# BlaineHeffron/WaveformML

Measured on AMD Instinct MI355X. Metric: waveforms/sec (LitPSD sparse-conv training step), higher is better.
Workload: dtype bf16; 1 GPU; SubMConv3d PSD net, 14x11 PMT grid x 256 samples, Cin=2 Cout=32, 256 events/rank/step, rulebook rebuilt every step; active_voxels_per_rank=84164, global_batch=256, parallelism=dp1, execution=hipgraph

## Files before the change

include/wfsparse.h:

```cpp
#ifndef WFSPARSE_H
#define WFSPARSE_H

#include <stddef.h>
#include <stdint.h>

#ifdef __cplusplus
extern "C" {
#endif

#define WFS_OK 0
#define WFS_EINVAL 1
#define WFS_EOVERFLOW 2
#define WFS_EHIP 3
#define WFS_EWORKSPACE 4

#define WFS_F32 0
#define WFS_BF16 1
#define WFS_F16 2

#define WFS_MAX_DIM 4

#define WFS_ABI_VERSION 6
int wfs_abi_version(void);
const char *wfs_last_error(void);
// ... 146 lines not shown

int wfs_to_dense_bwd_mapped(const void *dY, const uint32_t *ticket, const int32_t *slot_id, int64_t M,
                            const int64_t *m_dev, int32_t batch_size, int64_t V, int32_t C, void *dX, int32_t dtype,
                            void *stream);

int wfs_sparse_head_ok(int32_t batch, int64_t V, int32_t C, int32_t O, int32_t dtype);
size_t wfs_sparse_head_workspace_bytes(int32_t batch, int64_t V, int32_t C, int32_t O);
int wfs_sparse_head_fwd(const void *X, const uint32_t *ticket, const int32_t *slot_id, int64_t M,
                        const int64_t *m_dev, int32_t batch, int64_t V, int32_t C, const float *W,
                        const float *bias, int32_t O, float *Y, int32_t dtype, void *workspace,
                        size_t workspace_bytes, void *stream);
int wfs_sparse_head_bwd(const void *X, const float *G, const uint32_t *ticket, const int32_t *slot_id,
                        int64_t M, const int64_t *m_dev, int32_t batch, int64_t V, int32_t C, const float *W,
                        int32_t O, void *dX, float *dW, float *dB, int32_t dtype, void *workspace,
                        size_t workspace_bytes, wfs_dw_job *defer, void *stream);

size_t wfs_head_workspace_bytes(int64_t B, int64_t I, int32_t O);

int wfs_head_fwd(const void *X, int64_t B, int64_t I, const float *W, const float *bias, int32_t O,
                 float *Y, int32_t dtype, void *stream);

int wfs_head_bwd(const void *X, const float *G, int64_t B, int64_t I, const float *W, int32_t O,
                 void *dX, float *dW, float *dB, int32_t dtype, void *workspace, size_t workspace_bytes,
                 wfs_dw_job *defer, void *stream);



size_t wfs_tcn_lds_bytes(int32_t L, int32_t levels, int32_t backward);

int wfs_tcn_fwd(const void *X, int64_t N, int32_t L, const float *taps, const float *bias, int32_t levels,
// ... 86 lines not shown
```

waveformml_amd/_lib.py:

```python
import ctypes
import os

import torch

_HERE = os.path.dirname(os.path.abspath(__file__))
LIB_PATH = os.environ.get("WFS_LIB") or os.path.join(_HERE, "lib", "libwfsparse.so")

WFS_OK, WFS_EINVAL, WFS_EOVERFLOW, WFS_EHIP, WFS_EWORKSPACE = 0, 1, 2, 3, 4
WFS_F32, WFS_BF16, WFS_F16 = 0, 1, 2
WFS_MAX_DIM = 4
WFS_RNN_RELU, WFS_RNN_TANH = 0, 1
WFS_ABI_VERSION = 6
TIMER_GATHER_CONV, TIMER_GATHER_DW, TIMER_RULEBOOK, TIMER_CONV_BACKWARD = 0, 1, 2, 3

c_i32p = ctypes.POINTER(ctypes.c_int32)
c_i64p = ctypes.POINTER(ctypes.c_int64)
_vp, _i32, _i64, _sz = ctypes.c_void_p, ctypes.c_int32, ctypes.c_int64, ctypes.c_size_t


class Geometry(ctypes.Structure):
    _fields_ = [("ndim", _i32), ("batch_size", _i32), ("subm", _i32), ("K", _i32),
                ("spatial", _i32 * WFS_MAX_DIM), ("out_shape", _i32 * WFS_MAX_DIM),
                ("ksize", _i32 * WFS_MAX_DIM), ("stride", _i32 * WFS_MAX_DIM),
                ("padding", _i32 * WFS_MAX_DIM), ("dilation", _i32 * WFS_MAX_DIM),
# ... 57 lines not shown
                                       _i32, _vp, _vp, _vp, _vp, _sz, _i32, _vp, _vp]),
    "wfs_bn_relu_bwd": (ctypes.c_int, [_vp, _vp, _i64, _i32, _vp, _vp, _vp, _vp, _i32, _i32, _vp, _vp, _vp, _vp, _sz,
                                       _i32, _vp, _vp]),
    "wfs_rulebook_cell_map": (ctypes.c_int, [ctypes.POINTER(Geometry), _i64, _vp, ctypes.POINTER(_vp), ctypes.POINTER(_vp),
                                             c_i64p]),
    "wfs_to_dense_mapped": (ctypes.c_int, [_vp, _vp, _vp, _i64, _vp, _i32, _i64, _i32, _vp, _i32, _vp]),
    "wfs_to_dense_bwd_mapped": (ctypes.c_int, [_vp, _vp, _vp, _i64, _vp, _i32, _i64, _i32, _vp, _i32, _vp]),
    "wfs_to_dense": (ctypes.c_int, [_vp, _vp, _i64, _i32, c_i32p, _i32, _i32, _vp, _vp, _i32, _vp, _vp]),
    "wfs_to_dense_bwd": (ctypes.c_int, [_vp, _vp, _i64, _i32, c_i32p, _i32, _i32, _vp, _i32, _vp, _vp]),
    "wfs_sparse_head_ok": (ctypes.c_int, [_i32, _i64, _i32, _i32, _i32]),
    "wfs_sparse_head_workspace_bytes": (_sz, [_i32, _i64, _i32, _i32]),
    "wfs_sparse_head_fwd": (ctypes.c_int, [_vp, _vp, _vp, _i64, _vp, _i32, _i64, _i32, _vp, _vp, _i32, _vp, _i32, _vp, _sz,
                                           _vp]),
    "wfs_sparse_head_bwd": (ctypes.c_int, [_vp, _vp, _vp, _vp, _i64, _vp, _i32, _i64, _i32, _vp, _i32, _vp, _vp, _vp, _i32,
                                           _vp, _sz, ctypes.POINTER(DwJob), _vp]),
    "wfs_head_workspace_bytes": (_sz, [_i64, _i64, _i32]),
    "wfs_head_fwd": (ctypes.c_int, [_vp, _i64, _i64, _vp, _vp, _i32, _vp, _i32, _vp]),
    "wfs_head_bwd": (ctypes.c_int, [_vp, _vp, _i64, _i64, _vp, _i32, _vp, _vp, _vp, _i32, _vp, _sz, ctypes.POINTER(DwJob),
                                    _vp]),
    "wfs_tcn_lds_bytes": (_sz, [_i32, _i32, _i32]),
    "wfs_tcn_taps_fwd": (ctypes.c_int, [_vp, _i32, _i32, _vp, _vp, _vp]),
    "wfs_tcn_taps_bwd": (ctypes.c_int, [_vp, _i32, _i32, _vp, _i64, _vp]),
    "wfs_tcn_fwd": (ctypes.c_int, [_vp, _i64, _i32, _vp, _vp, _i32, _i32, _vp, _i32, ctypes.c_float, _vp, _vp]),
    "wfs_tcn_bwd": (ctypes.c_int, [_vp, _vp, _i64, _i32, _vp, _vp, _i32, _i32, _vp, _vp, _i32, ctypes.c_float, _vp,
                                    _vp]),
    "wfs_tcnc_ok": (ctypes.c_int, [_i32, c_i32p, _i32, _i32, _i32, _i32]),
    "wfs_tcnc_n_conv": (ctypes.c_int, [_i32, c_i32p, _i32, _i32]),
    "wfs_tcnc_weights_floats": (_sz, [_i32, c_i32p, _i32, _i32]),
    "wfs_tcnc_saved_floats": (_sz, [_i64, _i32, _i32, c_i32p, _i32]),
    "wfs_tcnc_bwd_workspace_floats": (_sz, [_i64, _i32, _i32, c_i32p, _i32, _i32]),
# ... 113 lines not shown
```

waveformml_amd/csrc/head.hip:

```cpp
#include "wfs_common.h"

namespace {
constexpr int TB = 256;
constexpr int MAXO = 8;

template <typename T>
__device__ __forceinline__ void load8(const T *p, float *v) {
    if constexpr (sizeof(T) == 4) {
        float4 a = *reinterpret_cast<const float4 *>(p), b = *reinterpret_cast<const float4 *>(p + 4);
        v[0] = a.x; v[1] = a.y; v[2] = a.z; v[3] = a.w; v[4] = b.x; v[5] = b.y; v[6] = b.z; v[7] = b.w;
    } else {
        uint4 u = *reinterpret_cast<const uint4 *>(p);
        wfs_unpack2<T>(u.x, v[0], v[1]);
        wfs_unpack2<T>(u.y, v[2], v[3]);
        wfs_unpack2<T>(u.z, v[4], v[5]);
        wfs_unpack2<T>(u.w, v[6], v[7]);
    }
}
template <typename T>
__device__ __forceinline__ void store8(T *p, const float *v) {
    if constexpr (sizeof(T) == 4) {
        *reinterpret_cast<float4 *>(p) = make_float4(v[0], v[1], v[2], v[3]);
        *reinterpret_cast<float4 *>(p + 4) = make_float4(v[4], v[5], v[6], v[7]);
    } else {
// ... 165 lines not shown
            for (int w = 0; w < TB / 64; ++w) v += sdb[w][threadIdx.x];
            dB[threadIdx.x] = v;
        }
    }
    long long e = (long long)blockIdx.x * TB + threadIdx.x;
    if (e >= OI) return;
    float s = 0.f;
    for (int c = 0; c < nchunk; ++c) s += part[(long long)c * OI + e];
    dW[e] = s;
}

int head_chunks(long long B) {
    long long c = (B + 31) / 32;
    return (int)(c < 1 ? 1 : (c > 16 ? 16 : c));
}
constexpr int XE_TB = 1024;
__global__ void __launch_bounds__(XE_TB) k_xent_mean(const float *__restrict__ Z, const long long *__restrict__ target,
                                                     long long B, int C, long long ignore_index,
                                                     float *__restrict__ loss, float *__restrict__ dZ) {
    __shared__ float sL[XE_TB];
    __shared__ float sN[XE_TB];
    float l = 0.f, n = 0.f;
    for (long long b = threadIdx.x; b < B; b += XE_TB) {
        const long long t = target[b];
        if (t == ignore_index || t < 0 || t >= C) continue;
        const float *z = Z + b * C;
        float m = z[0];
        for (int c = 1; c < C; ++c) m = fmaxf(m, z[c]);
        float se = 0.f;
        for (int c = 0; c < C; ++c) se += expf(z[c] - m);
        l += (m + logf(se)) - z[t];
        n += 1.f;
    }
    sL[threadIdx.x] = l;
    sN[threadIdx.x] = n;
    __syncthreads();
    for (int w = XE_TB / 2; w > 0; w >>= 1) {
        if ((int)threadIdx.x < w) {
            sL[threadIdx.x] += sL[threadIdx.x + w];
            sN[threadIdx.x] += sN[threadIdx.x + w];
        }
        __syncthreads();
    }
    const float cnt = sN[0];
    if (threadIdx.x == 0) *loss = sL[0] / cnt;
    if (!dZ) return;
    const float inv = cnt > 0.f ? 1.f / cnt : 0.f;
    for (long long b = threadIdx.x; b < B; b += XE_TB) {
        const long long t = target[b];
        const float *z = Z + b * C;
        float *d = dZ + b * C;
        if (t == ignore_index || t < 0 || t >= C) {
            for (int c = 0; c < C; ++c) d[c] = 0.f;
            continue;
        }
        float m = z[0];
        for (int c = 1; c < C; ++c) m = fmaxf(m, z[c]);
        float se = 0.f;
        for (int c = 0; c < C; ++c) se += expf(z[c] - m);
        const float r = inv / se;
        for (int c = 0; c < C; ++c) d[c] = expf(z[c] - m) * r - (c == t ? inv : 0.f);
    }
}

template <typename T, int O>
__global__ void __launch_bounds__(64) k_head_fwd_any(const T *__restrict__ X, const float *__restrict__ W,
                                                     const float *__restrict__ bias, float *__restrict__ Y, long long I) {
    const long long b = blockIdx.x;
    const int lane = threadIdx.x;
    float acc[O];
#pragma unroll
    for (int o = 0; o < O; ++o) acc[o] = 0.f;
    for (long long i = lane; i < I; i += 64) {
        const float x = wfs_ld(X + b * I + i);
#pragma unroll
        for (int o = 0; o < O; ++o) acc[o] = fmaf(x, W[o * I + i], acc[o]);
    }
// ... 188 lines not shown
```

waveformml_amd/csrc/shead.hip:

```cpp
#include <stdlib.h>

#include "wfs_common.h"

namespace {

constexpr int SH_CELLS = 64;
constexpr int SH_EVENTS = 16;

__device__ __forceinline__ long long valid_rows(long long R, const long long *r_dev) {
    long long v = r_dev ? *r_dev : R;
    return v < R ? v : R;
}

__device__ __forceinline__ void store8(float *p, const float *x) {
    *(float4 *)p = float4{x[0], x[1], x[2], x[3]};
    *(float4 *)(p + 4) = float4{x[4], x[5], x[6], x[7]};
}
template <typename H>
__device__ __forceinline__ void store8(H *p, const float *x) {
    uint4 v;
    v.x = wfs_pack2<H>(x[0], x[1]);
    v.y = wfs_pack2<H>(x[2], x[3]);
    v.z = wfs_pack2<H>(x[4], x[5]);
    v.w = wfs_pack2<H>(x[6], x[7]);
// ... 85 lines not shown
            for (int l = 0; l < 64; ++l) s += sT[l * TS + lane];
            sP[(cg * SH_EVENTS + e0) * O + lane] = s;
        }
        __builtin_amdgcn_wave_barrier();
    }
    __syncthreads();
    if (threadIdx.x < SH_EVENTS * O) {
        const int e = threadIdx.x / O;
        const int b = slice * SH_EVENTS + e;
        float s = 0.f;
        for (int g = 0; g < ncg; ++g) s += sP[g * SH_EVENTS * O + threadIdx.x];
        if (b < B) part[((long long)tile * B + b) * O + (threadIdx.x % O)] = s;
    }
}

__global__ void __launch_bounds__(256) k_shead_sum(const float *__restrict__ part, int ntiles, int B, int O,
                                                   const float *__restrict__ bias, float *__restrict__ Y) {
    const int i = blockIdx.x * 256 + threadIdx.x;
    if (i >= B * O) return;
    float s = bias ? bias[i % O] : 0.f;
    for (int t0 = 0; t0 < ntiles; t0 += 8) {
        float v[8];
#pragma unroll
        for (int t = 0; t < 8; ++t) v[t] = part[(long long)(t0 + t < ntiles ? t0 + t : ntiles - 1) * B * O + i];
#pragma unroll
        for (int t = 0; t < 8; ++t) s += t0 + t < ntiles ? v[t] : 0.f;
    }
    Y[i] = s;
}

template <typename H, int O>
__global__ void __launch_bounds__(512) k_shead_bwd(const H *__restrict__ X, const float *__restrict__ G,
                                                    const unsigned *__restrict__ ticket, const int *__restrict__ slot,
                                                    long long M, const long long *__restrict__ m_dev, int B, int V, int C,
                                                    const float *__restrict__ W, H *__restrict__ dX,
                                                    float *__restrict__ part, float *__restrict__ dB) {
    const int lane = threadIdx.x & 63, cg = threadIdx.x >> 6;
    const int tile = blockIdx.x, slice = blockIdx.y;
    const int cell = tile * SH_CELLS + lane;
    const bool in = cell < V;
    const int cc = in ? cell : V - 1;
    const long long Mv = valid_rows(M, m_dev);
    float w[O][8];
    if (dX) {
#pragma unroll
        for (int o = 0; o < O; ++o)
#pragma unroll
            for (int j = 0; j < 8; ++j) w[o][j] = W[((long long)o * C + cg * 8 + j) * V + cc];
    }
    int row[SH_EVENTS];
#pragma unroll
    for (int e = 0; e < SH_EVENTS; ++e) {
        const int b = slice * SH_EVENTS + e;
        const long long at = (long long)(b < B ? b : B - 1) * V + cc;
        const unsigned t = ticket[at];
        const int r = slot[at];
        row[e] = (in && b < B && t != 0xFFFFFFFFu && r >= 0 && r < Mv) ? r : -1;
    }
    float acc[O][8];
#pragma unroll
    for (int o = 0; o < O; ++o)
#pragma unroll
        for (int j = 0; j < 8; ++j) acc[o][j] = 0.f;
    constexpr int SH_BATCH = ShBatch<H>::n;
#pragma unroll
    for (int e0 = 0; e0 < SH_EVENTS; e0 += SH_BATCH) {
        Piece<H> q[SH_BATCH];
        float g[SH_BATCH][O];
#pragma unroll
        for (int i = 0; i < SH_BATCH; ++i) {
            if (part) q[i] = load_piece<H>(X + (long long)(row[e0 + i] >= 0 ? row[e0 + i] : 0) * C + cg * 8);
            const int b = slice * SH_EVENTS + e0 + i;
#pragma unroll
            for (int o = 0; o < O; ++o) g[i][o] = G[(long long)(b < B ? b : B - 1) * O + o];
        }
#pragma unroll
        for (int i = 0; i < SH_BATCH; ++i) {
            const int e = e0 + i;
            const bool act = row[e] >= 0;
            if (part) {
                float x[8];
                widen<H>(q[i], x);
#pragma unroll
                for (int o = 0; o < O; ++o) {
                    const float go = act ? g[i][o] : 0.f;
#pragma unroll
                    for (int j = 0; j < 8; ++j) acc[o][j] = fmaf(go, x[j], acc[o][j]);
                }
            }
            if (dX && act) {
                float d[8];
#pragma unroll
                for (int j = 0; j < 8; ++j) {
                    float t = 0.f;
#pragma unroll
                    for (int o = 0; o < O; ++o) t = fmaf(g[i][o], w[o][j], t);
                    d[j] = t;
                }
                store8(dX + (long long)row[e] * C + cg * 8, d);
            }
        }
    }
    if (part && in) {
        float *dst = part + (long long)slice * O * C * V;
#pragma unroll
        for (int o = 0; o < O; ++o)
#pragma unroll
            for (int j = 0; j < 8; ++j) dst[((long long)o * C + cg * 8 + j) * V + cell] = acc[o][j];
    }
    if (dB && tile == 0 && slice == 0 && cg == 0) {
#pragma unroll
        for (int o = 0; o < O; ++o) {
            float s = 0.f;
            for (int b = lane; b < B; b += 64) s += G[(long long)b * O + o];
#pragma unroll
            for (int d = 32; d >= 1; d >>= 1) s += __shfl_xor(s, d, 64);
            if (lane == 0) dB[o] = s;
        }
    }
}

inline size_t fwd_lds(int waves, int O) { return ((size_t)waves * 64 * ((8 * O) | 1) + (size_t)waves * SH_EVENTS * O) * sizeof(float); }
inline int sh_tiles(long long V) { return (int)wfs_cdiv(V, SH_CELLS); }
inline int sh_slices(int B) { return (int)wfs_cdiv(B, SH_EVENTS); }

}

extern "C" int wfs_sparse_head_ok(int32_t batch, int64_t V, int32_t C, int32_t O, int32_t dtype) {
    return batch >= 1 && batch <= 65535 * SH_EVENTS && V >= 1 && V < (1ll << 24) && C >= 8 && C <= 64 && C % 8 == 0 &&
           O >= 1 && O <= 4 && wfs_dtype_ok(dtype) && (long long)O * C * V < (1ll << 31) && (long long)batch * V < (1ll << 31);
}

extern "C" size_t wfs_sparse_head_workspace_bytes(int32_t batch, int64_t V, int32_t C, int32_t O) {
    const size_t fwd = (size_t)sh_tiles(V) * (size_t)batch * O * sizeof(float);
// ... 54 lines not shown
#define WFS_SHB(T)                                                                                                      \
    WFS_SH_DISPATCH(O, (k_shead_bwd<T, OO><<<grid, block, 0, stream>>>((const T *)X, G, ticket, slot_id, M, md, batch, (int)V, \
                                                                        C, W, (T *)dX, part, dB)))
    if (dtype == WFS_F32) { WFS_SHB(float); } else if (dtype == WFS_BF16) { WFS_SHB(wfs_bf16); } else { WFS_SHB(wfs_f16); }
#undef WFS_SHB
    WFS_LAUNCH_CHECK();
    if (!dW) return WFS_OK;
    const long long per = (long long)O * C * V;
    const wfs_dw_job job = {part, sh_slices(batch), per, 1, 1, 1, 0, dW};
    if (defer) {
        *defer = job;
        return WFS_OK;
    }
    return wfs_launch_dw_jobs(&job, 1, stream);
}
```

waveformml_amd/psd/lit.py:

```python
import logging

import torch
from torch import nn

from .config import DictionaryUtility, ModuleUtility


class LitPSD(nn.Module):
    def __init__(self, config, trial=None):
        super().__init__()
        self.trial = trial
        self.pylog = logging.getLogger(__name__)
        self.config = config
        self.n_type = config.system_config.n_type
        self.lr = config.optimize_config.lr
        self.modules_util = ModuleUtility(config.net_config.imports + config.dataset_config.imports +
                                          config.optimize_config.imports)
        self.model = self.modules_util.retrieve_class(config.net_config.net_class)(config)
        criterion_class = self.modules_util.retrieve_class(config.net_config.criterion_class)
        self.criterion = criterion_class(*config.net_config.criterion_params, reduction="mean")
        self.occlude_index = getattr(config.dataset_config, "occlude_index", None)
        self.softmax = nn.LogSoftmax(dim=1)
        self.logged = {}
        self.optimizer_parameters = None
# ... 40 lines not shown
            if not hasattr(oc, "scheduler_params"):
                raise IOError("Optimizer config has a learning scheduler class specified. You must also set "
                              "lr_schedule_parameters (dictionary of key value pairs).")
            scheduler = self.modules_util.retrieve_class(oc.scheduler_class)(
                optimizer, **DictionaryUtility.to_dict(oc.scheduler_params))
            return [optimizer], [scheduler]
        return optimizer

    def _loss(self, predictions, target):
        if predictions.is_cuda:
            from ..spconv import functional as Fsp
            if Fsp.can_fuse_cross_entropy(self.criterion, predictions, target):
                return Fsp.cross_entropy_mean(predictions, target, self.criterion.ignore_index)
        return self.criterion.forward(predictions, target)

    def training_step(self, batch, batch_idx):
        c, f, n_valid, target = self._unpack(batch)
        predictions = self._predict(c, f, target, n_valid)
        loss = self._loss(predictions, target)
        self.log("train_loss", loss, on_epoch=True, prog_bar=True, logger=True)
        return loss

    def validation_step(self, batch, batch_idx):
        c, f, n_valid, target = self._unpack(batch)
        predictions = self._predict(c, f, target, n_valid)
        loss = self.criterion.forward(predictions, target)
        pred = torch.argmax(self.softmax(predictions), dim=1)
        acc = (pred == target).float().mean()
        results = {"val_loss": loss, "val_acc": acc}
        self.log_dict(results, on_epoch=True, prog_bar=True, logger=True)
        return results

    def test_step(self, batch, batch_idx):
        c, f, n_valid, target = self._unpack(batch)
# ... 10 lines not shown
```

waveformml_amd/psd/net.py:

```python
import logging

import torch
from torch import nn

from .blocks import LinearBlock, SparseConv2DBlock, SparseConv2DPreserve
from .config import DictionaryUtility, ModuleUtility


class SPConvPreserveNet(nn.Module):

    def __init__(self, config):
        super().__init__()
        self.log = logging.getLogger(__name__)
        self.system_config = config.system_config
        self.net_config = config.net_config
        self.nsamples = self.system_config.n_samples
        self.ntype = self.system_config.n_type
        self.modules_util = ModuleUtility(self.net_config.imports)
        if "spconv" in self.modules_util.modules:
            self.spconv = self.modules_util.modules["spconv"]
        else:
            import waveformml_amd.spconv as sp
            self.spconv = sp
        hparams = DictionaryUtility.to_dict(self.net_config.hparams.conv_params)
# ... 34 lines not shown
        self.batch_size_hint = None
        self.batch_events = None
        self._build()
        net_type = getattr(self.net_config, "net_type", "2DConvolution")
        if net_type == "3DConvolution":
            self.ndim = 3
            self.spatial_size = [14, 11, int(self.nsamples)]
            self.register_buffer("permute_tensor", torch.LongTensor([3, 0, 1, 2]), persistent=False)
        else:
            if net_type != "2DConvolution":
                self.log.warning("Warning: unknown net_type in net_config: {}".format(net_type))
            self.ndim = 2
            self.spatial_size = [14, 11]
            self.register_buffer("permute_tensor", torch.LongTensor([2, 0, 1]), persistent=False)

    def forward(self, x, batch_size=None):
        coords, feats = x[0], x[1]
        if hasattr(self, "waveformLayer"):
            feats = self.waveformLayer(feats.unsqueeze(1)).squeeze(1)
        if batch_size is None:
            batch_size = getattr(self, "batch_size_hint", None)
        if batch_size is None:
            batch_size = int(coords[-1, -1]) + 1
        handed = getattr(self, "batch_first_indices", None)
        if handed is not None and handed[0] is coords:
            indices = handed[1]
        else:
            make = lambda: coords[:, self.permute_tensor].contiguous()
            reused = getattr(getattr(self.spconv, "ops", None), "reused", None)
            indices = reused("batch_first", coords, make) if reused is not None else make()
        st = self.spconv.SparseConvTensor(feats, indices, self.spatial_size,
                                          batch_size)
        if len(x) > 2 and x[2] is not None:
            st.n_valid = x[2]
        ev = getattr(self, "batch_events", None)
        if ev is not None and ev[0] is coords and handed is not None and handed[0] is coords:
            st.events = ev[1]
        return self._head(st)

    def _head(self, st):
        fsp = getattr(self.spconv, "functional", None)
        if fsp is not None and hasattr(fsp, "sparse_head") and hasattr(self.sparseModel, "run"):
            layers = list(self.linear)
            out = self.sparseModel.run(st, list(self.sparseModel._modules.values()), stop_before_dense=True)
            if hasattr(out, "features") and hasattr(out, "dense"):
                if fsp.can_use_sparse_head(out, layers):
                    self.head_route = "sparse_head"
                    return fsp.sparse_head(out, layers[0])
                out = out.dense()
        else:
            out = self.sparseModel(st)
        self.head_route = "dense"
        out = out.view(-1, self.n_linear)
        if fsp is not None and hasattr(fsp, "head_forward"):
            return fsp.head_forward(out, self.linear)
        head_dtype = next(self.linear.parameters()).dtype
        if out.dtype != head_dtype:
            out = out.to(head_dtype)
        return self.linear(out)

    def _build(self):
        if hasattr(self.net_config, "algorithm"):
# ... 64 lines not shown
        self.net_config = config.net_config
        self.nsamples = self.system_config.n_samples
        self.ntype = self.system_config.n_type
        self.modules_util = ModuleUtility(self.net_config.imports)
        self.spconv = self.modules_util.retrieve_module("spconv")
        self.sequence_class = self.modules_util.retrieve_class(self.net_config.sequence_class)
        self.batch_size_hint = None
        hparams = self.net_config.hparams
        params = DictionaryUtility.to_dict(hparams.wf_params) if hasattr(hparams, "wf_params") else {}
        self.waveformLayer = TemporalConvNet(1, [1] * hparams.n_dil, **params)
        self.voxelizer = Voxelizer(getattr(hparams, "threshold", 0.0))
        self._from_algorithm(self.net_config.algorithm)
        self.ndim = 3
        self.spatial_size = [14, 11, int(self.nsamples)]

    def forward(self, x, batch_size=None):
        coords, feats = x[0], x[1]
        n_valid = x[2] if len(x) > 2 else None
        if batch_size is None:
            batch_size = self.batch_size_hint
        if batch_size is None:
            batch_size = int(coords[-1, -1]) + 1
        values = self.waveformLayer(feats.unsqueeze(1)).squeeze(1)
        st = self.voxelizer(feats, values, coords, batch_size, self.spatial_size, self.spconv, n_valid)
        return self._head(st)
```

waveformml_amd/spconv/functional.py:

```python
import ctypes

import torch
from torch.autograd import Function

from .. import _lib

CONV, SUBM, INVERSE = 0, 1, 2

ACCOUNT = None


def _account(kind, table, R, rows_in, c_in, rows_out, c_out, K, cw_in, cw_out, esize):
    if ACCOUNT is None:
        return
    pairs = int((table >= 0).sum().item()) if table is not None else int(R)
    ACCOUNT.append(dict(kind=kind, pairs=pairs,
                        bytes=rows_in * c_in * esize + rows_out * c_out * esize + pairs * 8 + K * cw_in * cw_out * 4,
                        flops=2 * pairs * cw_in * cw_out))


def _features_ok(t):
    if not t.is_cuda:
        raise RuntimeError("waveformml_amd.spconv: features must be on the GPU (there is no CPU path)")
    return t.contiguous()
# ... 105 lines not shown


def register_grad_slots(flat_param, flat_grad):
    import weakref
    _GRAD_SLOTS[:] = [(p, g) for (p, g) in _GRAD_SLOTS if p() is not None and g() is not None]
    _GRAD_SLOTS.append((weakref.ref(flat_param), weakref.ref(flat_grad)))


_SLOTS_WRITTEN = set()


def reset_grad_slots():
    _SLOTS_WRITTEN.clear()


def grad_like(param, shape=None):
    shape = tuple(param.shape) if shape is None else tuple(shape)
    if (param is not None and param.is_cuda and param.dtype == torch.float32 and param.is_contiguous()
            and param.grad is None):
        for pref, gref in _GRAD_SLOTS:
            fp, fg = pref(), gref()
            if fp is None or fg is None or fp.device != param.device or fg.dtype != torch.float32:
                continue
            off = param.data_ptr() - fp.data_ptr()
            if 0 <= off and off + 4 * param.numel() <= 4 * fp.numel() and off % 4 == 0:
                slot = fg.data_ptr() + off
                if slot in _SLOTS_WRITTEN:
                    flush_deferred_dw()
                    _SHARED_SLOTS.add(slot)
                    break
                if not _SLOTS_WRITTEN:
                    try:
                        torch.autograd.Variable._execution_engine.queue_callback(reset_grad_slots)
                    except RuntimeError:
                        pass
                _SLOTS_WRITTEN.add(slot)
                return fg[off // 4: off // 4 + param.numel()].view(shape)
    return torch.empty(shape, dtype=torch.float32, device=param.device)


_DEFERRED_DW = None
_DEFERRED_SLOTS = set()
_SHARED_SLOTS = set()


def defer_dw(on):
    global _DEFERRED_DW
    _DEFERRED_DW = [] if on else None
    _DEFERRED_SLOTS.clear()
    _SHARED_SLOTS.clear()


# ... 495 lines not shown
        defer = _DEFERRED_DW is not None and dw is not None and dw._base is not None
        job = _lib.DwJob() if defer else None
        _lib.check(lib.wfs_sparse_head_bwd(_lib.ptr(features), _lib.ptr(g), ticket, slot, M, _lib.ptr(ctx.m_dev),
                                           ctx.batch_size, V, C, _lib.ptr(w), O, _lib.ptr(dx), _lib.ptr(dw), _lib.ptr(db),
                                           _lib.dtype_code(features), _lib.ptr(ws), ws.numel(),
                                           ctypes.byref(job) if defer else None, _lib.stream_ptr()))
        if defer and job.nslabs > 0:
            _DEFERRED_DW.append((job, ws))
        if want_db and db is None:
            db = g.sum(0)
        return (dx, (dw.to(weight.dtype) if dw is not None else None), (db.to(bias.dtype) if db is not None else None),
                None, None, None)


SPARSE_HEAD = __import__("os").environ.get("WFS_SPARSE_HEAD", "1") != "0"


def can_use_sparse_head(x, layers):
    if not SPARSE_HEAD or len(layers) != 1 or type(layers[0]) is not torch.nn.Linear:
        return False
    lin, f = layers[0], x.features
    cm = getattr(x, "cell_map", None)
    if cm is None or not f.is_cuda or f.dim() != 2 or f.shape[0] == 0 or lin.weight.dtype != torch.float32:
        return False
    if not (x.unique is True or x.n_valid is not None):
        return False
    V = 1
    for s_ in x.spatial_shape:
        V *= int(s_)
    C = int(f.shape[1])
    return bool(cm[3] == V and lin.in_features == C * V and f.dtype in (torch.float32, torch.bfloat16, torch.float16)
                and _lib.load().wfs_sparse_head_ok(int(x.batch_size), V, C, int(lin.out_features), _lib.dtype_code(f)))


def sparse_head(x, linear):
    return SparseHeadFunction.apply(x.features, linear.weight, linear.bias, x.cell_map, x.batch_size, x.n_valid)


def can_use_skinny_linear(linear, x):
    return (type(linear) is torch.nn.Linear and x.is_cuda and x.dim() == 2 and linear.out_features <= 8
            and ((x.shape[1] % 8 == 0 and x.shape[1] >= 1024) or x.shape[1] <= 4096)
            and x.dtype in (torch.float32, torch.bfloat16, torch.float16) and linear.weight.dtype == torch.float32)


def skinny_linear(x, linear):
    return SkinnyLinearFunction.apply(x, linear.weight, linear.bias)


class WideLinearFunction(Function):

    @staticmethod
    def forward(ctx, x, weight, bias):
        lib = _lib.load()
# ... 114 lines not shown
```

Before: 558,000 events/s.

## Fuse sparse linear head with cross-entropy loss and backward

Adds a fused path in which the sparse head's forward logits, the cross-entropy loss, the logit gradient and the head's dX/dW/dB are computed in a single sequence of kernels during the forward pass. Backward then only hands over the precomputed gradients, scaling them when the upstream gradient is not the unit loss gradient. This is meant to remove separate loss kernels, the second pass over the features in the head backward and several launches and intermediate tensors. In exchange it relies on the criterion being plain mean CrossEntropyLoss and adds complexity in gradient-slot handling and in when the deferred dW reduction runs.

```diff
diff --git a/include/wfsparse.h b/include/wfsparse.h
--- a/include/wfsparse.h
+++ b/include/wfsparse.h
@@ -184,6 +184,14 @@
                         int64_t M, const int64_t *m_dev, int32_t batch, int64_t V, int32_t C, const float *W,
                         int32_t O, void *dX, float *dW, float *dB, int32_t dtype, void *workspace,
                         size_t workspace_bytes, wfs_dw_job *defer, void *stream);
+
+int wfs_sparse_head_xent_ok(int32_t batch, int64_t V, int32_t C, int32_t O, int32_t dtype);
+size_t wfs_sparse_head_xent_workspace_bytes(int32_t batch, int64_t V, int32_t C, int32_t O);
+int wfs_sparse_head_xent(const void *X, const uint32_t *ticket, const int32_t *slot_id, int64_t M,
+                         const int64_t *m_dev, int32_t batch, int64_t V, int32_t C, const float *W,
+                         const float *bias, int32_t O, const int64_t *target, int64_t ignore_index, float *Y,
+                         float *loss, void *dX, int32_t want_dw, float *dB, int32_t dtype, void *workspace,
+                         size_t workspace_bytes, wfs_dw_job *job, void *stream);
 
 size_t wfs_head_workspace_bytes(int64_t B, int64_t I, int32_t O);
 
diff --git a/waveformml_amd/_lib.py b/waveformml_amd/_lib.py
--- a/waveformml_amd/_lib.py
+++ b/waveformml_amd/_lib.py
@@ -95,6 +95,10 @@
                                            _vp]),
     "wfs_sparse_head_bwd": (ctypes.c_int, [_vp, _vp, _vp, _vp, _i64, _vp, _i32, _i64, _i32, _vp, _i32, _vp, _vp, _vp, _i32,
                                            _vp, _sz, ctypes.POINTER(DwJob), _vp]),
+    "wfs_sparse_head_xent_ok": (ctypes.c_int, [_i32, _i64, _i32, _i32, _i32]),
+    "wfs_sparse_head_xent_workspace_bytes": (_sz, [_i32, _i64, _i32, _i32]),
+    "wfs_sparse_head_xent": (ctypes.c_int, [_vp, _vp, _vp, _i64, _vp, _i32, _i64, _i32, _vp, _vp, _i32, _vp, _i64, _vp,
+                                            _vp, _vp, _i32, _vp, _i32, _vp, _sz, ctypes.POINTER(DwJob), _vp]),
     "wfs_head_workspace_bytes": (_sz, [_i64, _i64, _i32]),
     "wfs_head_fwd": (ctypes.c_int, [_vp, _i64, _i64, _vp, _vp, _i32, _vp, _i32, _vp]),
     "wfs_head_bwd": (ctypes.c_int, [_vp, _vp, _i64, _i64, _vp, _i32, _vp, _vp, _vp, _i32, _vp, _sz, ctypes.POINTER(DwJob),
diff --git a/waveformml_amd/csrc/head.hip b/waveformml_amd/csrc/head.hip
--- a/waveformml_amd/csrc/head.hip
+++ b/waveformml_amd/csrc/head.hip
@@ -1,4 +1,5 @@
 #include "wfs_common.h"
+#include "wfs_xent.h"
 
 namespace {
 constexpr int TB = 256;
@@ -203,7 +204,6 @@
     long long c = (B + 31) / 32;
     return (int)(c < 1 ? 1 : (c > 16 ? 16 : c));
 }
-constexpr int XE_TB = 1024;
 __global__ void __launch_bounds__(XE_TB) k_xent_mean(const float *__restrict__ Z, const long long *__restrict__ target,
                                                      long long B, int C, long long ignore_index,
                                                      float *__restrict__ loss, float *__restrict__ dZ) {
@@ -212,44 +212,19 @@
     float l = 0.f, n = 0.f;
     for (long long b = threadIdx.x; b < B; b += XE_TB) {
         const long long t = target[b];
-        if (t == ignore_index || t < 0 || t >= C) continue;
-        const float *z = Z + b * C;
-        float m = z[0];
-        for (int c = 1; c < C; ++c) m = fmaxf(m, z[c]);
-        float se = 0.f;
-        for (int c = 0; c < C; ++c) se += expf(z[c] - m);
-        l += (m + logf(se)) - z[t];
+        if (!xent_counts(t, C, ignore_index)) continue;
+        l += xent_row_loss(Z + b * C, C, t);
         n += 1.f;
     }
     sL[threadIdx.x] = l;
     sN[threadIdx.x] = n;
     __syncthreads();
-    for (int w = XE_TB / 2; w > 0; w >>= 1) {
-        if ((int)threadIdx.x < w) {
-            sL[threadIdx.x] += sL[threadIdx.x + w];
-            sN[threadIdx.x] += sN[threadIdx.x + w];
-        }
-        __syncthreads();
-    }
+    xent_tree(sL, sN);
     const float cnt = sN[0];
     if (threadIdx.x == 0) *loss = sL[0] / cnt;
     if (!dZ) return;
     const float inv = cnt > 0.f ? 1.f / cnt : 0.f;
-    for (long long b = threadIdx.x; b < B; b += XE_TB) {
-        const long long t = target[b];
-        const float *z = Z + b * C;
-        float *d = dZ + b * C;
-        if (t == ignore_index || t < 0 || t >= C) {
-            for (int c = 0; c < C; ++c) d[c] = 0.f;
-            continue;
-        }
-        float m = z[0];
-        for (int c = 1; c < C; ++c) m = fmaxf(m, z[c]);
-        float se = 0.f;
-        for (int c = 0; c < C; ++c) se += expf(z[c] - m);
-        const float r = inv / se;
-        for (int c = 0; c < C; ++c) d[c] = expf(z[c] - m) * r - (c == t ? inv : 0.f);
-    }
+    for (long long b = threadIdx.x; b < B; b += XE_TB) xent_row_grad(Z + b * C, C, target[b], ignore_index, inv, dZ + b * C);
 }
 
 template <typename T, int O>
diff --git a/waveformml_amd/csrc/shead.hip b/waveformml_amd/csrc/shead.hip
--- a/waveformml_amd/csrc/shead.hip
+++ b/waveformml_amd/csrc/shead.hip
@@ -1,6 +1,7 @@
 #include <stdlib.h>
 
 #include "wfs_common.h"
+#include "wfs_xent.h"
 
 namespace {
 
@@ -123,19 +124,216 @@
     }
 }
 
+__device__ __forceinline__ float shead_logit(const float *__restrict__ part, int ntiles, int B, int O, int i, float s) {
+    for (int t0 = 0; t0 < ntiles; t0 += 24) {
+        float v[24];
+#pragma unroll
+        for (int t = 0; t < 24; ++t) v[t] = part[(long long)(t0 + t < ntiles ? t0 + t : ntiles - 1) * B * O + i];
+#pragma unroll
+        for (int g = 0; g < 24; g += 8) {
+            if (t0 + g < ntiles) {
+#pragma unroll
+                for (int t = g; t < g + 8; ++t) s += t0 + t < ntiles ? v[t] : 0.f;
+            }
+        }
+    }
+    return s;
+}
+
 __global__ void __launch_bounds__(256) k_shead_sum(const float *__restrict__ part, int ntiles, int B, int O,
                                                    const float *__restrict__ bias, float *__restrict__ Y) {
     const int i = blockIdx.x * 256 + threadIdx.x;
     if (i >= B * O) return;
-    float s = bias ? bias[i % O] : 0.f;
-    for (int t0 = 0; t0 < ntiles; t0 += 8) {
-        float v[8];
-#pragma unroll
-        for (int t = 0; t < 8; ++t) v[t] = part[(long long)(t0 + t < ntiles ? t0 + t : ntiles - 1) * B * O + i];
-#pragma unroll
-        for (int t = 0; t < 8; ++t) s += t0 + t < ntiles ? v[t] : 0.f;
-    }
-    Y[i] = s;
+    Y[i] = shead_logit(part, ntiles, B, O, i, bias ? bias[i % O] : 0.f);
+}
+
+struct ShXent {
+    const float *fpart;
+    const float *bias;
+    const long long *target;
+    long long ignore_index;
+    float *Y;
+    float *loss;
+    float *dZ;
+};
+
+template <int O>
+__device__ __forceinline__ void shead_db(const float *G, int B, int lane, float *__restrict__ dB) {
+#pragma unroll
+    for (int o = 0; o < O; ++o) {
+        float s = 0.f;
+        for (int b = lane; b < B; b += 64) s += G[(long long)b * O + o];
+#pragma unroll
+        for (int d = 32; d >= 1; d >>= 1) s += __shfl_xor(s, d, 64);
+        if (lane == 0) dB[o] = s;
+    }
+}
+
+template <int O>
+__device__ __forceinline__ void shead_xent_batch(int B, int ntiles, float *__restrict__ dB, const ShXent &xe) {
+    __shared__ float sL[XE_TB];
+    __shared__ float sN[XE_TB];
+    for (int vt = threadIdx.x; vt < XE_TB; vt += blockDim.x) {
+        float n = 0.f;
+        for (int b = vt; b < B; b += XE_TB) n += xent_counts(xe.target[b], O, xe.ignore_index) ? 1.f : 0.f;
+        sN[vt] = n;
+        sL[vt] = 0.f;
+    }
+    __syncthreads();
+    xent_tree(sN, nullptr);
+    const float cnt = sN[0];
+    const float inv = cnt > 0.f ? 1.f / cnt : 0.f;
+    for (int vt = threadIdx.x; vt < XE_TB; vt += blockDim.x) {
+        float l = 0.f;
+        for (int b = vt; b < B; b += XE_TB) {
+            float z[O], d[O];
+#pragma unroll
+            for (int o = 0; o < O; ++o) {
+                z[o] = shead_logit(xe.fpart, ntiles, B, O, b * O + o, xe.bias ? xe.bias[o] : 0.f);
+                xe.Y[(long long)b * O + o] = z[o];
+            }
+            const long long t = xe.target[b];
+            xent_row_grad(z, O, t, xe.ignore_index, inv, d);
+#pragma unroll
+            for (int o = 0; o < O; ++o) xe.dZ[(long long)b * O + o] = d[o];
+            if (!xent_counts(t, O, xe.ignore_index)) continue;
+            l += xent_row_loss(z, O, t);
+        }
+        sL[vt] = l;
+    }
+    __syncthreads();
+    xent_tree(sL, nullptr);
+    if (threadIdx.x == 0) *xe.loss = sL[0] / cnt;
+    if (dB && threadIdx.x < 64) shead_db<O>(xe.dZ, B, (int)threadIdx.x, dB);
+}
+
+template <typename H, int O, bool FUSED>
+__device__ __forceinline__ void shead_bwd_body(const H *__restrict__ X, const float *__restrict__ G,
+                                               const unsigned *__restrict__ ticket, const int *__restrict__ slot,
+                                               long long M, const long long *__restrict__ m_dev, int B, int V, int C,
+                                               const float *__restrict__ W, H *__restrict__ dX, float *__restrict__ part,
+                                               float *__restrict__ dB, const ShXent &xe) {
+    const int lane = threadIdx.x & 63, cg = threadIdx.x >> 6;
+    const int tile = blockIdx.x, slice = blockIdx.y;
+    if constexpr (FUSED) {
+        if (slice * SH_EVENTS >= B) {
+            if (tile == 0) shead_xent_batch<O>(B, (int)gridDim.x, dB, xe);
+            return;
+        }
+    }
+    const int cell = tile * SH_CELLS + lane;
+    const bool in = cell < V;
+    const int cc = in ? cell : V - 1;
+    const long long Mv = valid_rows(M, m_dev);
+    float w[O][8];
+    if (dX) {
+#pragma unroll
+        for (int o = 0; o < O; ++o)
+#pragma unroll
+            for (int j = 0; j < 8; ++j) w[o][j] = W[((long long)o * C + cg * 8 + j) * V + cc];
+    }
+    int row[SH_EVENTS];
+#pragma unroll
+    for (int e = 0; e < SH_EVENTS; ++e) {
+        const int b = slice * SH_EVENTS + e;
+        const long long at = (long long)(b < B ? b : B - 1) * V + cc;
+        const unsigned t = ticket[at];
+        const int r = slot[at];
+        row[e] = (in && b < B && t != 0xFFFFFFFFu && r >= 0 && r < Mv) ? r : -1;
+    }
+    float acc[O][8];
+#pragma unroll
+    for (int o = 0; o < O; ++o)
+#pragma unroll
+        for (int j = 0; j < 8; ++j) acc[o][j] = 0.f;
+    constexpr int SH_BATCH = ShBatch<H>::n;
+    Piece<H> q[SH_BATCH];
+    __shared__ float sG[FUSED ? SH_EVENTS * O : 1];
+    if constexpr (FUSED) {
+        if (part) {
+#pragma unroll
+            for (int i = 0; i < SH_BATCH; ++i) q[i] = load_piece<H>(X + (long long)(row[i] >= 0 ? row[i] : 0) * C + cg * 8);
+        }
+        if (cg == 0) {
+            const int e = lane < SH_EVENTS * O ? lane / O : 0;
+            const int be = slice * SH_EVENTS + e;
+            const int bi = be < B ? be : B - 1;
+            const float z1 = shead_logit(xe.fpart, (int)gridDim.x, B, O, bi * O + lane % O, xe.bias ? xe.bias[lane % O] : 0.f);
+            const int bt = slice * SH_EVENTS + (lane < SH_EVENTS ? lane : 0);
+            const long long t = xe.target[bt < B ? bt : B - 1];
+            int n = 0;
+            for (int b0 = lane; b0 < B; b0 += 256) {
+                long long tb[4];
+#pragma unroll
+                for (int u = 0; u < 4; ++u) tb[u] = xe.target[b0 + 64 * u < B ? b0 + 64 * u : B - 1];
+#pragma unroll
+                for (int u = 0; u < 4; ++u) n += (b0 + 64 * u < B && xent_counts(tb[u], O, xe.ignore_index)) ? 1 : 0;
+            }
+#pragma unroll
+            for (int d = 32; d >= 1; d >>= 1) n += __shfl_xor(n, d, 64);
+            const float cnt = (float)n;
+            const float inv = cnt > 0.f ? 1.f / cnt : 0.f;
+            float z[O], d[O];
+#pragma unroll
+            for (int o = 0; o < O; ++o) z[o] = __shfl(z1, (lane < SH_EVENTS ? lane : 0) * O + o, 64);
+            xent_row_grad(z, O, t, xe.ignore_index, inv, d);
+            if (lane < SH_EVENTS) {
+#pragma unroll
+                for (int o = 0; o < O; ++o) sG[lane * O + o] = bt < B ? d[o] : 0.f;
+            }
+            }
+        __syncthreads();
+    }
+#pragma unroll
+    for (int e0 = 0; e0 < SH_EVENTS; e0 += SH_BATCH) {
+        float g[SH_BATCH][O];
+#pragma unroll
+        for (int i = 0; i < SH_BATCH; ++i) {
+            if (part && !(FUSED && e0 == 0))
+                q[i] = load_piece<H>(X + (long long)(row[e0 + i] >= 0 ? row[e0 + i] : 0) * C + cg * 8);
+            const int b = slice * SH_EVENTS + e0 + i;
+#pragma unroll
+            for (int o = 0; o < O; ++o) {
+                if constexpr (FUSED) g[i][o] = sG[(e0 + i) * O + o];
+                else g[i][o] = G[(long long)(b < B ? b : B - 1) * O + o];
+            }
+        }
+#pragma unroll
+        for (int i = 0; i < SH_BATCH; ++i) {
+            const int e = e0 + i;
+            const bool act = row[e] >= 0;
+            if (part) {
+                float x[8];
+                widen<H>(q[i], x);
+#pragma unroll
+                for (int o = 0; o < O; ++o) {
+                    const float go = act ? g[i][o] : 0.f;
+#pragma unroll
+                    for (int j = 0; j < 8; ++j) acc[o][j] = fmaf(go, x[j], acc[o][j]);
+                }
+            }
+            if (dX && act) {
+                float d[8];
+#pragma unroll
+                for (int j = 0; j < 8; ++j) {
+                    float t = 0.f;
+#pragma unroll
+                    for (int o = 0; o < O; ++o) t = fmaf(g[i][o], w[o][j], t);
+                    d[j] = t;
+                }
+                store8(dX + (long long)row[e] * C + cg * 8, d);
+            }
+        }
+    }
+    if (part && in) {
+        float *dst = part + (long long)slice * O * C * V;
+#pragma unroll
+        for (int o = 0; o < O; ++o)
+#pragma unroll
+            for (int j = 0; j < 8; ++j) dst[((long long)o * C + cg * 8 + j) * V + cell] = acc[o][j];
+    }
+    if constexpr (FUSED) return;
+    if (dB && tile == 0 && slice == 0 && cg == 0) shead_db<O>(G, B, lane, dB);
 }
 
 template <typename H, int O>
@@ -144,89 +342,16 @@
                                                     long long M, const long long *__restrict__ m_dev, int B, int V, int C,
                                                     const float *__restrict__ W, H *__restrict__ dX,
                                                     float *__restrict__ part, float *__restrict__ dB) {
-    const int lane = threadIdx.x & 63, cg = threadIdx.x >> 6;
-    const int tile = blockIdx.x, slice = blockIdx.y;
-    const int cell = tile * SH_CELLS + lane;
-    const bool in = cell < V;
-    const int cc = in ? cell : V - 1;
-    const long long Mv = valid_rows(M, m_dev);
-    float w[O][8];
-    if (dX) {
-#pragma unroll
-        for (int o = 0; o < O; ++o)
-#pragma unroll
-            for (int j = 0; j < 8; ++j) w[o][j] = W[((long long)o * C + cg * 8 + j) * V + cc];
-    }
-    int row[SH_EVENTS];
-#pragma unroll
-    for (int e = 0; e < SH_EVENTS; ++e) {
-        const int b = slice * SH_EVENTS + e;
-        const long long at = (long long)(b < B ? b : B - 1) * V + cc;
-        const unsigned t = ticket[at];
-        const int r = slot[at];
-        row[e] = (in && b < B && t != 0xFFFFFFFFu && r >= 0 && r < Mv) ? r : -1;
-    }
-    float acc[O][8];
-#pragma unroll
-    for (int o = 0; o < O; ++o)
-#pragma unroll
-        for (int j = 0; j < 8; ++j) acc[o][j] = 0.f;
-    constexpr int SH_BATCH = ShBatch<H>::n;
-#pragma unroll
-    for (int e0 = 0; e0 < SH_EVENTS; e0 += SH_BATCH) {
-        Piece<H> q[SH_BATCH];
-        float g[SH_BATCH][O];
-#pragma unroll
-        for (int i = 0; i < SH_BATCH; ++i) {
-            if (part) q[i] = load_piece<H>(X + (long long)(row[e0 + i] >= 0 ? row[e0 + i] : 0) * C + cg * 8);
-            const int b = slice * SH_EVENTS + e0 + i;
-#pragma unroll
-            for (int o = 0; o < O; ++o) g[i][o] = G[(long long)(b < B ? b : B - 1) * O + o];
-        }
-#pragma unroll
-        for (int i = 0; i < SH_BATCH; ++i) {
-            const int e = e0 + i;
-            const bool act = row[e] >= 0;
-            if (part) {
-                float x[8];
-                widen<H>(q[i], x);
-#pragma unroll
-                for (int o = 0; o < O; ++o) {
-                    const float go = act ? g[i][o] : 0.f;
-#pragma unroll
-                    for (int j = 0; j < 8; ++j) acc[o][j] = fmaf(go, x[j], acc[o][j]);
-                }
-            }
-            if (dX && act) {
-                float d[8];
-#pragma unroll
-                for (int j = 0; j < 8; ++j) {
-                    float t = 0.f;
-#pragma unroll
-                    for (int o = 0; o < O; ++o) t = fmaf(g[i][o], w[o][j], t);
-                    d[j] = t;
-                }
-                store8(dX + (long long)row[e] * C + cg * 8, d);
-            }
-        }
-    }
-    if (part && in) {
-        float *dst = part + (long long)slice * O * C * V;
-#pragma unroll
-        for (int o = 0; o < O; ++o)
-#pragma unroll
-            for (int j = 0; j < 8; ++j) dst[((long long)o * C + cg * 8 + j) * V + cell] = acc[o][j];
-    }
-    if (dB && tile == 0 && slice == 0 && cg == 0) {
-#pragma unroll
-        for (int o = 0; o < O; ++o) {
-            float s = 0.f;
-            for (int b = lane; b < B; b += 64) s += G[(long long)b * O + o];
-#pragma unroll
-            for (int d = 32; d >= 1; d >>= 1) s += __shfl_xor(s, d, 64);
-            if (lane == 0) dB[o] = s;
-        }
-    }
+    shead_bwd_body<H, O, false>(X, G, ticket, slot, M, m_dev, B, V, C, W, dX, part, dB, ShXent{});
+}
+
+template <typename H, int O>
+__global__ void __launch_bounds__(512) k_shead_xent_bwd(const H *__restrict__ X, const unsigned *__restrict__ ticket,
+                                                         const int *__restrict__ slot, long long M,
+                                                         const long long *__restrict__ m_dev, int B, int V, int C,
+                                                         const float *__restrict__ W, H *__restrict__ dX,
+                                                         float *__restrict__ part, float *__restrict__ dB, ShXent xe) {
+    shead_bwd_body<H, O, true>(X, nullptr, ticket, slot, M, m_dev, B, V, C, W, dX, part, dB, xe);
 }
 
 inline size_t fwd_lds(int waves, int O) { return ((size_t)waves * 64 * ((8 * O) | 1) + (size_t)waves * SH_EVENTS * O) * sizeof(float); }
@@ -311,3 +436,57 @@
     }
     return wfs_launch_dw_jobs(&job, 1, stream);
 }
+
+constexpr int SHX_MAX_BATCH = 1 << 16;
+
+static size_t shx_align(size_t n) { return (n + 255) & ~(size_t)255; }
+static size_t shx_fwd_bytes(int batch, long long V, int O) { return shx_align((size_t)sh_tiles(V) * (size_t)batch * O * sizeof(float)); }
+static size_t shx_bwd_bytes(int batch, long long V, int C, int O) {
+    return shx_align((size_t)sh_slices(batch) * (size_t)O * C * (size_t)V * sizeof(float));
+}
+
+extern "C" int wfs_sparse_head_xent_ok(int32_t batch, int64_t V, int32_t C, int32_t O, int32_t dtype) {
+    return wfs_sparse_head_ok(batch, V, C, O, dtype) && batch <= SHX_MAX_BATCH;
+}
+
+extern "C" size_t wfs_sparse_head_xent_workspace_bytes(int32_t batch, int64_t V, int32_t C, int32_t O) {
+    return shx_bwd_bytes(batch, V, C, O) + shx_fwd_bytes(batch, V, O) + shx_align((size_t)batch * O * sizeof(float));
+}
+
+extern "C" int wfs_sparse_head_xent(const void *X, const uint32_t *ticket, const int32_t *slot_id, int64_t M,
+                                    const int64_t *m_dev, int32_t batch, int64_t V, int32_t C, const float *W,
+                                    const float *bias, int32_t O, const int64_t *target, int64_t ignore_index, float *Y,
+                                    float *loss, void *dX, int32_t want_dw, float *dB, int32_t dtype, void *workspace,
+                                    size_t workspace_bytes, wfs_dw_job *job, void *stream_) {
+    hipStream_t stream = (hipStream_t)stream_;
+    WFS_REQUIRE(wfs_sparse_head_xent_ok(batch, V, C, O, dtype), WFS_EINVAL,
+                "wfs_sparse_head_xent: shape not covered (wfs_sparse_head_xent_ok)");
+    WFS_REQUIRE(X && ticket && slot_id && W && target && Y && loss && workspace, WFS_EINVAL, "NULL device pointer");
+    WFS_REQUIRE(!want_dw || job, WFS_EINVAL, "the dW partials are summed by the job handed back");
+    WFS_REQUIRE(!dB || want_dw, WFS_EINVAL, "dB comes with dW");
+    WFS_REQUIRE(workspace_bytes >= wfs_sparse_head_xent_workspace_bytes(batch, V, C, O), WFS_EWORKSPACE, "workspace too small");
+    WFS_REQUIRE(M >= 0, WFS_EINVAL, "M");
+    if (job) *job = wfs_dw_job{nullptr, 0, 0, 0, 0, 0, 0, nullptr};
+    float *part = (float *)workspace;
+    float *fpart = (float *)((char *)workspace + shx_bwd_bytes(batch, V, C, O));
+    float *dZ = (float *)((char *)fpart + shx_fwd_bytes(batch, V, O));
+    const dim3 grid((unsigned)sh_tiles(V), (unsigned)sh_slices(batch)), block(64 * (C / 8));
+    const long long *md = (const long long *)m_dev;
+    const dim3 xgrid(grid.x, grid.y + 1);
+    const ShXent xe = {fpart, bias, (const long long *)target, ignore_index, Y, loss, dZ};
+#define WFS_SHXF(T)                                                                                                     \
+    WFS_SH_DISPATCH(O, (k_shead_fwd<T, OO><<<grid, block, fwd_lds(C / 8, OO), stream>>>((const T *)X, ticket, slot_id, M, md, \
+                                                                                         batch, (int)V, C, W, fpart)))
+    if (dtype == WFS_F32) { WFS_SHXF(float); } else if (dtype == WFS_BF16) { WFS_SHXF(wfs_bf16); } else { WFS_SHXF(wfs_f16); }
+#undef WFS_SHXF
+    WFS_LAUNCH_CHECK();
+#define WFS_SHXB(T)                                                                                                     \
+    WFS_SH_DISPATCH(O, (k_shead_xent_bwd<T, OO><<<xgrid, block, 0, stream>>>((const T *)X, ticket, slot_id, M, md, batch,   \
+                                                                             (int)V, C, W, (T *)dX,                      \
+                                                                             want_dw ? part : nullptr, dB, xe)))
+    if (dtype == WFS_F32) { WFS_SHXB(float); } else if (dtype == WFS_BF16) { WFS_SHXB(wfs_bf16); } else { WFS_SHXB(wfs_f16); }
+#undef WFS_SHXB
+    WFS_LAUNCH_CHECK();
+    if (want_dw) *job = wfs_dw_job{part, sh_slices(batch), (long long)O * C * V, 1, 1, 1, 0, nullptr};
+    return WFS_OK;
+}
diff --git a/waveformml_amd/csrc/wfs_xent.h b/waveformml_amd/csrc/wfs_xent.h
--- /dev/null
+++ b/waveformml_amd/csrc/wfs_xent.h
@@ -0,0 +1,46 @@
+#ifndef WFS_XENT_H
+#define WFS_XENT_H
+
+#include <hip/hip_runtime.h>
+
+constexpr int XE_TB = 1024;
+
+__device__ __forceinline__ bool xent_counts(long long t, int C, long long ignore_index) {
+    return !(t == ignore_index || t < 0 || t >= C);
+}
+
+__device__ __forceinline__ float xent_row_loss(const float *z, int C, long long t) {
+    float m = z[0];
+    for (int c = 1; c < C; ++c) m = fmaxf(m, z[c]);
+    float se = 0.f;
+    for (int c = 0; c < C; ++c) se += expf(z[c] - m);
+    float zt = z[0];
+    for (int c = 1; c < C; ++c) zt = c == t ? z[c] : zt;
+    return (m + logf(se)) - zt;
+}
+
+__device__ __forceinline__ void xent_row_grad(const float *z, int C, long long t, long long ignore_index, float inv,
+                                              float *d) {
+    if (!xent_counts(t, C, ignore_index)) {
+        for (int c = 0; c < C; ++c) d[c] = 0.f;
+        return;
+    }
+    float m = z[0];
+    for (int c = 1; c < C; ++c) m = fmaxf(m, z[c]);
+    float se = 0.f;
+    for (int c = 0; c < C; ++c) se += expf(z[c] - m);
+    const float r = inv / se;
+    for (int c = 0; c < C; ++c) d[c] = expf(z[c] - m) * r - (c == t ? inv : 0.f);
+}
+
+__device__ __forceinline__ void xent_tree(float *sL, float *sN) {
+    for (int w = XE_TB / 2; w > 0; w >>= 1) {
+        for (int i = threadIdx.x; i < w; i += blockDim.x) {
+            sL[i] += sL[i + w];
+            if (sN) sN[i] += sN[i + w];
+        }
+        __syncthreads();
+    }
+}
+
+#endif
diff --git a/waveformml_amd/psd/lit.py b/waveformml_amd/psd/lit.py
--- a/waveformml_amd/psd/lit.py
+++ b/waveformml_amd/psd/lit.py
@@ -4,6 +4,7 @@
 from torch import nn
 
 from .config import DictionaryUtility, ModuleUtility
+from .net import SPConvNet
 
 
 class LitPSD(nn.Module):
@@ -78,10 +79,20 @@
                 return Fsp.cross_entropy_mean(predictions, target, self.criterion.ignore_index)
         return self.criterion.forward(predictions, target)
 
+    def _predict_with_loss(self, c, f, target, n_valid=None):
+        if c.is_cuda and isinstance(self.model, SPConvNet):
+            from ..spconv import functional as Fsp
+            if Fsp.head_loss_fusable(self.criterion, self.training):
+                self.model.batch_size_hint = int(target.shape[0])
+                predictions, loss = self.model([c, f, n_valid] if n_valid is not None else [c, f],
+                                               xent=(target, self.criterion.ignore_index))
+                return predictions, (loss if loss is not None else self._loss(predictions, target))
+        predictions = self._predict(c, f, target, n_valid)
+        return predictions, self._loss(predictions, target)
+
     def training_step(self, batch, batch_idx):
         c, f, n_valid, target = self._unpack(batch)
-        predictions = self._predict(c, f, target, n_valid)
-        loss = self._loss(predictions, target)
+        _predictions, loss = self._predict_with_loss(c, f, target, n_valid)
         self.log("train_loss", loss, on_epoch=True, prog_bar=True, logger=True)
         return loss
 
diff --git a/waveformml_amd/psd/net.py b/waveformml_amd/psd/net.py
--- a/waveformml_amd/psd/net.py
+++ b/waveformml_amd/psd/net.py
@@ -72,7 +72,7 @@
             self.spatial_size = [14, 11]
             self.register_buffer("permute_tensor", torch.LongTensor([2, 0, 1]), persistent=False)
 
-    def forward(self, x, batch_size=None):
+    def forward(self, x, batch_size=None, xent=None):
         coords, feats = x[0], x[1]
         if hasattr(self, "waveformLayer"):
             feats = self.waveformLayer(feats.unsqueeze(1)).squeeze(1)
@@ -94,9 +94,16 @@
         ev = getattr(self, "batch_events", None)
         if ev is not None and ev[0] is coords and handed is not None and handed[0] is coords:
             st.events = ev[1]
-        return self._head(st)
-
-    def _head(self, st):
+        return self._head(st, xent)
+
+    def _head(self, st, xent=None):
+        self.head_fused = False
+        out = self._run_head(st, xent)
+        if xent is None:
+            return out
+        return out if self.head_fused else (out, None)
+
+    def _run_head(self, st, xent):
         fsp = getattr(self.spconv, "functional", None)
         if fsp is not None and hasattr(fsp, "sparse_head") and hasattr(self.sparseModel, "run"):
             layers = list(self.linear)
@@ -104,6 +111,10 @@
             if hasattr(out, "features") and hasattr(out, "dense"):
                 if fsp.can_use_sparse_head(out, layers):
                     self.head_route = "sparse_head"
+                    if (xent is not None and hasattr(fsp, "sparse_head_xent")
+                            and fsp.can_use_sparse_head_xent(out, layers[0], xent[0])):
+                        self.head_fused = True
+                        return fsp.sparse_head_xent(out, layers[0], xent[0], xent[1])
                     return fsp.sparse_head(out, layers[0])
                 out = out.dense()
         else:
@@ -198,7 +209,7 @@
         self.ndim = 3
         self.spatial_size = [14, 11, int(self.nsamples)]
 
-    def forward(self, x, batch_size=None):
+    def forward(self, x, batch_size=None, xent=None):
         coords, feats = x[0], x[1]
         n_valid = x[2] if len(x) > 2 else None
         if batch_size is None:
@@ -207,4 +218,4 @@
             batch_size = int(coords[-1, -1]) + 1
         values = self.waveformLayer(feats.unsqueeze(1)).squeeze(1)
         st = self.voxelizer(feats, values, coords, batch_size, self.spatial_size, self.spconv, n_valid)
-        return self._head(st)
+        return self._head(st, xent)
diff --git a/waveformml_amd/spconv/functional.py b/waveformml_amd/spconv/functional.py
--- a/waveformml_amd/spconv/functional.py
+++ b/waveformml_amd/spconv/functional.py
@@ -143,28 +143,42 @@
     _SLOTS_WRITTEN.clear()
 
 
+def _slots_of(param):
+    if not (param is not None and param.is_cuda and param.dtype == torch.float32 and param.is_contiguous()
+            and param.grad is None):
+        return
+    for pref, gref in _GRAD_SLOTS:
+        fp, fg = pref(), gref()
+        if fp is None or fg is None or fp.device != param.device or fg.dtype != torch.float32:
+            continue
+        off = param.data_ptr() - fp.data_ptr()
+        if 0 <= off and off + 4 * param.numel() <= 4 * fp.numel() and off % 4 == 0:
+            yield fg, off
+
+
+def peek_grad_slot(param, shape=None):
+    for fg, off in _slots_of(param):
+        if fg.data_ptr() + off in _SLOTS_WRITTEN:
+            return None
+        return fg[off // 4: off // 4 + param.numel()].view(tuple(param.shape) if shape is None else tuple(shape))
+    return None
+
+
 def grad_like(param, shape=None):
     shape = tuple(param.shape) if shape is None else tuple(shape)
-    if (param is not None and param.is_cuda and param.dtype == torch.float32 and param.is_contiguous()
-            and param.grad is None):
-        for pref, gref in _GRAD_SLOTS:
-            fp, fg = pref(), gref()
-            if fp is None or fg is None or fp.device != param.device or fg.dtype != torch.float32:
-                continue
-            off = param.data_ptr() - fp.data_ptr()
-            if 0 <= off and off + 4 * param.numel() <= 4 * fp.numel() and off % 4 == 0:
-                slot = fg.data_ptr() + off
-                if slot in _SLOTS_WRITTEN:
-                    flush_deferred_dw()
-                    _SHARED_SLOTS.add(slot)
-                    break
-                if not _SLOTS_WRITTEN:
-                    try:
-                        torch.autograd.Variable._execution_engine.queue_callback(reset_grad_slots)
-                    except RuntimeError:
-                        pass
-                _SLOTS_WRITTEN.add(slot)
-                return fg[off // 4: off // 4 + param.numel()].view(shape)
+    for fg, off in _slots_of(param):
+        slot = fg.data_ptr() + off
+        if slot in _SLOTS_WRITTEN:
+            flush_deferred_dw()
+            _SHARED_SLOTS.add(slot)
+            break
+        if not _SLOTS_WRITTEN:
+            try:
+                torch.autograd.Variable._execution_engine.queue_callback(reset_grad_slots)
+            except RuntimeError:
+                pass
+        _SLOTS_WRITTEN.add(slot)
+        return fg[off // 4: off // 4 + param.numel()].view(shape)
     return torch.empty(shape, dtype=torch.float32, device=param.device)
 
 
@@ -690,6 +704,7 @@
 
 
 SPARSE_HEAD = __import__("os").environ.get("WFS_SPARSE_HEAD", "1") != "0"
+SPARSE_HEAD_XENT = __import__("os").environ.get("WFS_SPARSE_HEAD_XENT", "1") != "0"
 
 
 def can_use_sparse_head(x, layers):
@@ -713,6 +728,98 @@
     return SparseHeadFunction.apply(x.features, linear.weight, linear.bias, x.cell_map, x.batch_size, x.n_valid)
 
 
+class SparseHeadXentFunction(Function):
+
+    @staticmethod
+    def forward(ctx, features, weight, bias, cell_map, batch_size, m_dev, target, ignore_index):
+        lib = _lib.load()
+        features = _features_ok(features)
+        target = target.contiguous()
+        M, C = features.shape
+        ticket, slot, _keep, V = cell_map
+        B, O, dev = int(batch_size), int(weight.shape[0]), features.device
+        w = weight.detach().float().contiguous()
+        b = None if bias is None else bias.detach().float().contiguous()
+        y = torch.empty((B, O), dtype=torch.float32, device=dev)
+        loss = torch.empty((1,), dtype=torch.float32, device=dev)
+        want_dw = bool(ctx.needs_input_grad[1])
+        want_db = bias is not None and bool(ctx.needs_input_grad[2])
+        dx = _rows((M, C), features, m_dev) if ctx.needs_input_grad[0] else None
+        db = None
+        if want_db:
+            db = peek_grad_slot(bias, (O,))
+            if db is None:
+                db = torch.empty((O,), dtype=torch.float32, device=dev)
+        ws = torch.empty((int(lib.wfs_sparse_head_xent_workspace_bytes(B, V, C, O)),), dtype=torch.uint8, device=dev)
+        job = _lib.DwJob()
+        _lib.check(lib.wfs_sparse_head_xent(_lib.ptr(features), ticket, slot, M, _lib.ptr(m_dev), B, V, C, _lib.ptr(w),
+                                            _lib.ptr(b), O, _lib.ptr(target), int(ignore_index), _lib.ptr(y),
+                                            _lib.ptr(loss), _lib.ptr(dx), 1 if (want_dw or want_db) else 0, _lib.ptr(db),
+                                            _lib.dtype_code(features), _lib.ptr(ws), ws.numel(), ctypes.byref(job),
+                                            _lib.stream_ptr()))
+        ctx.save_for_backward(weight, bias)
+        ctx.stash = (dx, db, job if want_dw else None, ws)
+        ctx.dw_shape = (O, C * V)
+        ctx.mark_non_differentiable(y)
+        ctx.set_materialize_grads(False)
+        return y, loss.reshape(())
+
+    @staticmethod
+    def backward(ctx, _grad_logits, grad_output):
+        if ctx.stash is None:
+            raise RuntimeError("the fused head's gradients were handed over by an earlier backward(): run the forward again")
+        weight, bias = ctx.saved_tensors
+        if grad_output is None:
+            return (None,) * 8
+        (dx, db_made, job, ws), ctx.stash = ctx.stash, None
+        unit = _UNIT_LOSS_GRAD.get(grad_output.device)
+        scale = None if (unit is not None and grad_output.data_ptr() == unit.data_ptr()) else grad_output
+        dw = db = None
+        if job is not None:
+            dw = grad_like(weight, ctx.dw_shape)
+            job.dW = dw.data_ptr()
+            if scale is None and _DEFERRED_DW is not None and dw._base is not None:
+                _DEFERRED_DW.append((job, ws))
+            else:
+                _lib.check(_lib.load().wfs_dw_reduce_jobs(ctypes.byref(job), 1, _lib.stream_ptr()))
+                if scale is not None:
+                    dw.mul_(scale)
+        if db_made is not None:
+            db = grad_like(bias, tuple(db_made.shape))
+            if db.data_ptr() == db_made.data_ptr():
+                if scale is not None:
+                    db.mul_(scale)
+            elif db._base is None:
+                db = db_made if scale is None else db_made * scale
+            else:
+                torch.mul(db_made, 1.0 if scale is None else scale, out=db)
+        if dx is not None and scale is not None:
+            dx = dx * scale
+        return (dx, (dw.to(weight.dtype) if dw is not None else None), (db.to(bias.dtype) if db is not None else None),
+                None, None, None, None, None)
+
+
+def head_loss_fusable(criterion, training, grad_enabled=None):
+    if grad_enabled is None:
+        grad_enabled = torch.is_grad_enabled()
+    return bool(SPARSE_HEAD_XENT and training and grad_enabled and type(criterion) is torch.nn.CrossEntropyLoss
+                and criterion.reduction == "mean" and criterion.weight is None
+                and getattr(criterion, "label_smoothing", 0.0) == 0.0)
+
+
+def can_use_sparse_head_xent(x, linear, target):
+    f = x.features
+    return bool(torch.is_tensor(target) and target.is_cuda and target.device == f.device and target.dtype == torch.int64
+                and target.dim() == 1 and int(target.shape[0]) == int(x.batch_size)
+                and _lib.load().wfs_sparse_head_xent_ok(int(x.batch_size), int(x.cell_map[3]), int(f.shape[1]),
+                                                        int(linear.out_features), _lib.dtype_code(f)))
+
+
+def sparse_head_xent(x, linear, target, ignore_index=-100):
+    return SparseHeadXentFunction.apply(x.features, linear.weight, linear.bias, x.cell_map, x.batch_size, x.n_valid,
+                                        target, ignore_index)
+
+
 def can_use_skinny_linear(linear, x):
     return (type(linear) is torch.nn.Linear and x.is_cuda and x.dim() == 2 and linear.out_features <= 8
             and ((x.shape[1] % 8 == 0 and x.shape[1] >= 1024) or x.shape[1] <= 4096)
```

New measurement: 564,900 events/s, median of 6. 1.01x the previous value.
